# klasmodin/quflow

Measured on AMD Instinct MI355X. Metric: isospectral timesteps/sec at N=1024 (1 GPU) + ensemble steps/sec at 1/2/4/8 GPUs, higher is better.
Workload: dtype f64

## Files before the change

quflow_amd/csrc/api_isomp.hip:

```cpp
#include <cmath>
#include <cstdarg>
#include <cstdio>
#include <cstdlib>
#include <cstring>
#include <limits>
#include <chrono>
#include <type_traits>
#include <utility>

#include "qf_api.h"

namespace {

#ifndef QF_RUN_AHEAD
#define QF_RUN_AHEAD 3
#endif

template <class S> constexpr bool is_c64 = std::is_same<S, qf_c64>::value;

template <class S> S *ws(qf_ctx *ctx)
{
    if constexpr (is_c64<S>) return ctx->c64;
    else return ctx;
}
// ... 92 lines not shown

int select_second_product_c64(qf_ctx *ctx)
{
    qf_c64 *f = ctx->c64;
    f->tri = false;
    if (f->tri_allowed && ctx->gemm_tri_allowed && (qf_c64_tile(ctx) == 32 || ctx->N % 64 == 0) && ctx->N >= 64) {
        QF_TRY(check_skew(ctx, f));
        if (f->w_skew_known) {
            QF_TRY(qf_c64_tri_alloc(ctx));
            f->tri = true;
        }
    }
    return QF_OK;
}

bool triangle_product(const qf_ctx *ctx) { return (ctx->gemm_tri || ctx->gemm_tri32) && (!ctx->gemm_i8 || ctx->gemm_i8_first); }
bool triangle_product(const qf_c64 *f) { return f->tri; }

template <class S> int begin_increment(qf_ctx *ctx, S *w, bool carry)
{
    const size_t mbytes = (size_t)ctx->N * ctx->N * sizeof(*w->W);
    if (carry) {
        if (w->dw_cur != 0)
            QF_HIP(hipMemcpyAsync(w->dW[0], w->dW[w->dw_cur], mbytes, hipMemcpyDeviceToDevice, ctx->stream));
        QF_TRY(qf_launch_lincomb(ctx, 1, w->W, 1, w->dW[0], 0, w->Whalf));
    } else {
        QF_HIP(hipMemsetAsync(w->dW[0], 0, mbytes, ctx->stream));
        QF_HIP(hipMemcpyAsync(w->Whalf, w->W, mbytes, hipMemcpyDeviceToDevice, ctx->stream));
    }
    return QF_OK;
}

template <class S> int enqueue_iterations(qf_ctx *ctx, int step, int first, int count, double vareps)
// ... 35 lines not shown
    d.ticket = ctx->ticket + 402;
    return d;
}

template <class S> int enqueue_iterations_fused(qf_ctx *ctx, int step, int first, int count, double vareps, bool last_step)
{
    S *w = ws<S>(ctx);
    const bool defer = !is_c64<S> && ctx->defer;
    const qf_decide dec = defer ? deferred_decision(ctx) : qf_decide();
    for (int i = first; i < first + count; ++i) {
        qf_guard g;
        g.state = ctx->state;
        g.step = step;
        g.iter = i;
        g.alt = w->Whalf2;
        {
            prof_scope p(ctx, QF_KERNEL_POISSON);
            if constexpr (is_c64<S>) QF_TRY(launch_solve(ctx, w->Whalf, w->Phalf, vareps, g));
            else QF_TRY(launch_solve(ctx, w->Whalf, w->Phalf, vareps, g, defer ? &dec : nullptr));
        }
        {
            prof_scope p(ctx, QF_KERNEL_GEMM1);
            QF_TRY(launch_gemm(ctx, w->Phalf, w->Whalf, w->PW, nullptr, g));
        }
        {
            prof_scope p(ctx, QF_KERNEL_GEMM2);
            const auto ep = epilogue_of(w, true);
            g.alt = nullptr;
            if constexpr (is_c64<S>) {
                if (w->tri) QF_TRY(qf_launch_cgemm_tri(ctx, w->PW, w->Phalf, &ep, g));
                else QF_TRY(qf_launch_cgemm(ctx, w->PW, w->Phalf, nullptr, &ep, g));
            } else {
                QF_TRY(qf_launch_zgemm(ctx, w->PW, w->Phalf, nullptr, &ep, g));
            }
        }
    }
    if (defer && last_step && count > 0) QF_TRY(qf_launch_decide(ctx, dec));
    return QF_OK;
}

int enqueue_iterations_fused_i8(qf_ctx *ctx, int step, int first, int count, double vareps)
{
// ... 66 lines not shown
            jobs.j[0].X = ctx->PW;
            jobs.j[0].planes = ctx->oz_planes[3];
            jobs.j[0].scale = ctx->oz_scale[3];
            QF_TRY(qf_launch_oz_slice(ctx, jobs, g, ctx->oz_digits2));
        }
        {
            prof_scope p(ctx, QF_KERNEL_GEMM2);
            const qf_epilogue ep = epilogue_of(ctx, true);
            QF_TRY(qf_launch_oz_gemm(ctx, ctx->oz_planes[3], ctx->oz_scale[3], ctx->oz_planes[0], ctx->oz_scale[0], nullptr,
                                     &ep, g, ctx->oz_digits2, ctx->oz_digits2 ? ctx->oz_digits : 0));
        }
    }
    return QF_OK;
}

template <class S> struct fused_run {
    qf_ctx *ctx = nullptr;
    int steps = 0, minit = 1, maxit = 1;
    double vareps = 0.0;
    int pred = 1, pred0 = 1;
    std::vector<int> enq_iters;
    int known = 0, enq = 0;
    bool first_seen = false;
    bool aborted = false;
    unsigned long long idle_polls = 0;

    int enqueue(int step, int first, int count)
    {
        if constexpr (!is_c64<S>)
            if (ctx->gemm_i8) return enqueue_iterations_fused_i8(ctx, step, first, count, vareps);
        return enqueue_iterations_fused<S>(ctx, step, first, count, vareps, step == steps - 1);
    }
    bool cold_start = true;
    void begin(qf_ctx *c, int steps_, int minit_, int maxit_, double vareps_)
    {
        ctx = c;
        cold_start = ws<S>(c)->increment_is_zero;
        steps = steps_;
        minit = minit_;
        maxit = maxit_;
        vareps = vareps_;
        pred = ctx->pred_iters;
        if (pred < minit) pred = minit;
        if (pred > maxit) pred = maxit;
        pred0 = ctx->pred_first_iters > 0 ? ctx->pred_first_iters : pred + 1;
        if (pred0 < pred) pred0 = pred;
        if (pred0 > maxit) pred0 = maxit;
        enq_iters.assign((size_t)steps + 1, 0);
        known = enq = 0;
        first_seen = false;
        aborted = false;
        idle_polls = 0;
    }
    bool done() const { return known >= steps; }
    int pump()
    {
        if (done()) return QF_OK;
        while (enq < steps && enq - known < QF_RUN_AHEAD) {
            const int n = (enq == 0 && cold_start) ? pred0 : pred;
            QF_TRY(enqueue(enq, 0, n));
            enq_iters[enq] = n;
            ++enq;
        }
        volatile qf_host_record *rec = ctx->host_rec;
        unsigned long long p = __atomic_load_n(&rec->progress, __ATOMIC_ACQUIRE);
        int ps = (int)(p >> 32), pi = (int)(p & 0xffffffffull);
        if (ps >= QF_STEP_ABORTED) {
            aborted = true;
            known = steps;
            return QF_OK;
        }
        if (!(ps > known || (ps == known && pi >= enq_iters[known]))) {
            if (++idle_polls > (1ull << 22)) {
                QF_HIP(hipStreamSynchronize(ctx->stream));
                p = __atomic_load_n(&rec->progress, __ATOMIC_ACQUIRE);
                ps = (int)(p >> 32);
                pi = (int)(p & 0xffffffffull);
                if (ps >= QF_STEP_ABORTED) {
// ... 16 lines not shown
                first_seen = true;
                if (it >= minit && it <= maxit) ctx->pred_first_iters = it;
            } else if (it >= minit && it <= maxit) {
                pred = it;
            }
            known = ps < enq ? ps : enq;
            if (done()) ctx->pred_iters = pred;
            return QF_OK;
        }
        const int have = enq_iters[known];
        if (have >= maxit) {
            qf_set_error("qf_isomp: step %d did not close after maxit=%d iterations (internal error)", known, maxit);
            return QF_ERR_STATE;
        }
        QF_TRY(enqueue(known, have, maxit - have));
        enq_iters[known] = maxit;
        enq = known + 1;
        if (pred < maxit) pred += 1;
        return QF_OK;
    }
};

bool poll_yields()
{
    static const int mode = [] {
        const char *e = getenv("QUFLOW_HIP_POLL");
        return (e && strcmp(e, "yield") == 0) ? 1 : 0;
    }();
    return mode == 1;
}

inline void poll_relax()
{
    if (poll_yields()) {
// ... 56 lines not shown
int reset_after_abort(qf_ctx *ctx)
{
    if (!ctx->needs_reset) return QF_OK;
    QF_HIP(hipMemsetAsync(ctx->ticket, 0, 704 * sizeof(unsigned), ctx->stream));
    if (ctx->sk_flags) QF_HIP(hipMemsetAsync(ctx->sk_flags + (ctx->sk_slots > 0 ? ctx->sk_slots : ctx->num_cus), 0, 16 * sizeof(unsigned), ctx->stream));
    if (ctx->t32_arrive) {
        const size_t nt = (size_t)(ctx->N + 31) / 32;
        QF_HIP(hipMemsetAsync(ctx->t32_arrive, 0, nt * (nt + 1) / 2 * sizeof(unsigned), ctx->stream));
    }
    if (ctx->c64 && ctx->c64->tri_arrive)
        QF_HIP(hipMemsetAsync(ctx->c64->tri_arrive, 0, ctx->c64->tri_arrive_count * sizeof(unsigned), ctx->stream));
    ctx->needs_reset = false;
    return QF_OK;
}

template <class S> int fused_enter(qf_ctx *ctx, double dt, double tol, int minit, int maxit, bool carry)
{
    S *w = ws<S>(ctx);
    const size_t mbytes = (size_t)ctx->N * ctx->N * sizeof(*w->W);
    const bool tol_on_device = tol < 0;
    const double tol_factor = tol_on_device ? mach_eps<S>(true) * dt / qf_hbar(ctx->N) : 0.0;
    QF_TRY(reset_after_abort(ctx));
    if constexpr (is_c64<S>) {
        QF_TRY(select_second_product_c64(ctx));
    } else {
        QF_TRY(select_second_product(ctx));
        ctx->defer = ctx->defer_allowed && !ctx->gemm_i8 && ctx->gemm_tri32 && ctx->N <= 512;
    }
    w->increment_is_zero = !carry;
    w->increment_valid = true;
    volatile qf_host_record *rec = ctx->host_rec;
    rec->progress = 0ull;
    rec->step_index = 0;
    rec->fault = 0;
    rec->nonfinite = 0;
    __atomic_thread_fence(__ATOMIC_SEQ_CST);
    if (is_c64<S> || carry) {
        if (tol_on_device) QF_TRY(qf_launch_norm_inf(ctx, w->W, ctx->scalars));
        QF_TRY(begin_increment(ctx, w, carry));
        QF_TRY(qf_launch_state_init(ctx, tol, minit, maxit, tol_on_device ? ctx->scalars : nullptr, tol_factor));
    } else {
        QF_TRY(qf_launch_call_begin(ctx, tol, minit, maxit, tol_on_device ? 1 : 0, tol_factor));
    }
    if (!w->W2) QF_HIP(hipMalloc((void **)&w->W2, mbytes));
    if (!w->Whalf2) QF_HIP(hipMalloc((void **)&w->Whalf2, mbytes));
    if constexpr (!is_c64<S>)
        if (ctx->gemm_i8) QF_TRY(qf_oz_alloc(ctx));
    return QF_OK;
}

template <class S> int fused_leave(qf_ctx *ctx, int steps, qf_isomp_stats *stats_out)
{
    S *w = ws<S>(ctx);
    volatile qf_host_record *rec = ctx->host_rec;
    const int w_parity = steps > 0 ? rec->w_parity : 0, wh_sel = steps > 0 ? rec->wh_sel : 0;
    w->dw_cur = steps > 0 ? rec->dw_parity : 0;
    if (w_parity) std::swap(w->W, w->W2);
    if (wh_sel) std::swap(w->Whalf, w->Whalf2);
    if (triangle_product(w) && steps > 0) {
        QF_TRY(qf_launch_mirror_lower(ctx, w->W));
        QF_TRY(qf_launch_mirror_lower(ctx, w->dW[w->dw_cur]));
    }
    if constexpr (!is_c64<S>)
        if (ctx->diag_at_exit) {
            QF_TRY(qf_enqueue_diagnostics(ctx));
            ctx->diag_valid = true;
        }
    QF_HIP(hipStreamSynchronize(ctx->stream));
    if (rec->nonfinite) {
        qf_set_error("array must not contain infs or NaNs");
        ctx->needs_reset = true;
        w->increment_valid = false;
        ctx->diag_valid = false;
        rec->nonfinite = 0;
        return QF_ERR_NONFINITE;
    }
    if (steps > 0 && rec->step_index != steps) {
        qf_set_error("qf_isomp: device completed %d of %d steps (internal error)", rec->step_index, steps);
        return QF_ERR_STATE;
    }
// ... 46 lines not shown
    auto now = [] { return std::chrono::steady_clock::now(); };
    auto ms_since = [&](std::chrono::steady_clock::time_point t) {
        return std::chrono::duration<double, std::milli>(now() - t).count();
    };
    const auto t_entry = now();
    double t_tol = 0, t_sel = 0, t_init = 0, t_loop = 0, t_waitmax = 0, t_waitat = 0, t_enqmax = 0, t_enqat = 0;
    int waitstep = -1, enqstep = -1;
    S *w = ws<S>(ctx);
    const int N = ctx->N;
    const size_t mbytes = (size_t)N * N * sizeof(*w->W);
    const double hb = qf_hbar(N);
    const double vareps = dt / (2 * hb);
    const bool carry = carry_increment && w->increment_valid && !reinitialize;

    if (ctx->fused_allowed && !compsum && !reinitialize) {
        int rc = fused_enter<S>(ctx, dt, tol, minit, maxit, carry);
        t_init = ms_since(t_entry);
        if (rc == QF_OK) rc = run_fused<S>(ctx, steps, minit, maxit, vareps);
        const double t_run = ms_since(t_entry);
        if (rc == QF_OK) rc = fused_leave<S>(ctx, steps, stats_out);
        if (rc != QF_OK) fused_abort(ctx);
        if (dbg)
            fprintf(stderr, "[quflow_hip] %s %d steps (fused step end): init %.3f run %.3f end %.3f ms (cumulative); %lld iterations\n",
                    is_c64<S> ? "qf_c64_isomp" : "qf_isomp", steps, t_init, t_run, ms_since(t_entry),
                    (long long)ctx->host_rec->total_iterations);
        return rc;
    }

    if (tol < 0) {
        double nrm = 0.0;
        QF_TRY(qf_launch_norm_inf(ctx, w->W, ctx->scalars));
// ... 154 lines not shown
        for (int q = 0; q < k; ++q) {
            const int rc = isomp_impl<S>(ctxs[q], dt, steps, tol, minit, maxit, 0, 0, stats_out ? stats_out + q : nullptr, false);
            if (rc != QF_OK) {
                mark_failed(q);
                if (first_rc == QF_OK) first_rc = rc;
            }
        }
        return first_rc;
    }
    auto abort_all = [&](int rc) {
        for (int q = 0; q < k; ++q) fused_abort(ctxs[q]);
        return rc;
    };
    std::vector<fused_run<S>> runs((size_t)k);
    for (int r = 0; r < k; ++r) {
        const int rc = fused_enter<S>(ctxs[r], dt, tol, minit, maxit, false);
        if (rc != QF_OK) return abort_all(rc);
        runs[r].begin(ctxs[r], steps, minit, maxit, dt / (2 * qf_hbar(ctxs[r]->N)));
    }
    for (;;) {
        bool all = true;
        for (int r = 0; r < k; ++r) {
            if (runs[r].done()) continue;
            const int rc = runs[r].pump();
            if (rc != QF_OK) return abort_all(rc);
            all = all && runs[r].done();
        }
        if (all) break;
        poll_relax();
    }
    int first_rc = QF_OK;
// ... 35 lines not shown
    } else {
        QF_TRY(qf_launch_cgemm(ctx, f->PW, f->Phalf, nullptr, &ep));
        QF_TRY(qf_launch_sum_rowpart(ctx, f->rowpart, f->rowpart_tiles, ctx->rowsum));
    }
    QF_HIP(hipMemcpyAsync(dW_new_host, f->dW[1], bytes, hipMemcpyDeviceToHost, ctx->stream));
    QF_HIP(hipMemcpyAsync(Whalf_new_host, f->Whalf, bytes, hipMemcpyDeviceToHost, ctx->stream));
    QF_HIP(hipMemcpyAsync(rowsum_host, ctx->rowsum, (size_t)N * sizeof(double), hipMemcpyDeviceToHost, ctx->stream));
    QF_HIP(hipStreamSynchronize(ctx->stream));
    return QF_OK;
}

}

int qf_rowpart_slots(const qf_ctx *ctx) { return ctx->gemm_tri ? ctx->N / 64 : ctx->gemm_tri32 ? (ctx->N + 31) / 32 : ctx->rowpart_tiles; }

int qf_enqueue_diagnostics(qf_ctx *ctx)
{
    QF_TRY(qf_launch_solve(ctx, ctx->poisson, ctx->W, ctx->stage, 1.0, 1));
    QF_TRY(qf_launch_inner2(ctx, ctx->W, ctx->stage, ctx->scalars + 2));
    QF_HIP(hipMemcpyAsync(ctx->host_scalars, ctx->scalars + 2, 2 * sizeof(double), hipMemcpyDeviceToHost, ctx->stream));
    return QF_OK;
}

int qf_isomp_multi(qf_ctx **ctxs, int k, double dt, int steps, double tol, int minit, int maxit, qf_isomp_stats *stats_out)
{
    return isomp_multi<qf_ctx>(ctxs, k, dt, steps, tol, minit, maxit, stats_out);
}

int qf_c64_isomp_multi(qf_ctx **ctxs, int k, double dt, int steps, double tol, int minit, int maxit, qf_isomp_stats *stats_out)
{
    return isomp_multi<qf_c64>(ctxs, k, dt, steps, tol, minit, maxit, stats_out);
}

int qf_isomp(qf_ctx *ctx, double dt, int steps, double tol, int minit, int maxit, int compsum,
// ... 135 lines not shown
```

quflow_amd/csrc/elementwise.hip:

```cpp
#include "qf_internal.h"

#pragma clang fp contract(off)

namespace {

constexpr int TU = 32;

__device__ __forceinline__ cplx make_c(double re, double im) { return make_double2(re, im); }
__device__ __forceinline__ float2 make_c(float re, float im) { return make_float2(re, im); }
__device__ __forceinline__ double modulus_d(cplx z) { return hypot(z.x, z.y); }
__device__ __forceinline__ double modulus_d(float2 z) { return (double)hypotf(z.x, z.y); }
__device__ __forceinline__ double re_dot_d(cplx a, cplx b) { return a.x * b.x + a.y * b.y; }
__device__ __forceinline__ double re_dot_d(float2 a, float2 b) { return (double)(a.x * b.x + a.y * b.y); }

__device__ void qf_step_advance(qf_dev_state *state, qf_host_record *rec, const qf_guard &guard)
{
    const bool mine = state->step_index == guard.step;
    const bool complete = mine && (state->step_done != 0 || state->iters_this_step >= state->maxit);
    int incomplete = 0;
    if (complete) {
        if (!state->step_done) state->number_of_maxit += 1;
        rec->last_step_iters = state->iters_this_step;
        state->step_index += 1;
        state->iters_this_step = 0;
// ... 174 lines not shown
    const int bi = blockIdx.y, bj = blockIdx.x;
    if (bj > bi) return;
    const int i0 = bi * TU, j0 = bj * TU;
    for (int r = ty; r < TU; r += 8) {
        const int gj = j0 + r, gi = i0 + tx;
        C tv = make_c(R(0), R(0));
        if (gj < N && gi < N) tv = X[(size_t)gj * N + gi];
        Ts[r][tx] = tv;
    }
    __syncthreads();
    for (int r = ty; r < TU; r += 8) {
        const int gi = i0 + r, gj = j0 + tx;
        if (gi < N && gj < N && gj < gi) {
            const C t = Ts[tx][r];
            X[(size_t)gi * N + gj] = make_c(-t.x, t.y);
        }
    }
}

__global__ __launch_bounds__(256) void k_magnetic_fix(int N, const cplx *__restrict__ BTP, const cplx *__restrict__ BT,
                                                       cplx *__restrict__ dW, const cplx *__restrict__ dW_old,
                                                       const cplx *__restrict__ W, cplx *__restrict__ Whalf,
                                                       double *__restrict__ rowpart)
{
    __shared__ cplx Tp[TU][TU + 1], Tb[TU][TU + 1];
    __shared__ double rs[8][TU];
    const int tx = threadIdx.x & 31, ty = threadIdx.x >> 5;
    const int i0 = blockIdx.y * TU, j0 = blockIdx.x * TU;
    for (int r = ty; r < TU; r += 8) {
        const int gj = j0 + r, gi = i0 + tx;
// ... 272 lines not shown
    __hip_atomic_store(&rec->seq, 0ull, __ATOMIC_RELEASE, __HIP_MEMORY_SCOPE_SYSTEM);
}

__device__ __forceinline__ bool last_block_of_launch(unsigned *t, int bid, int nb)
{
    const int g = bid >> 5, ng = (nb + 31) >> 5;
    const int gsize = (g == ng - 1) ? nb - (g << 5) : 32;
    asm volatile("s_waitcnt vmcnt(0)" ::: "memory");
    if (__hip_atomic_fetch_add(t + 1 + g, 1u, __ATOMIC_RELAXED, __HIP_MEMORY_SCOPE_AGENT) != (unsigned)(gsize - 1)) return false;
    __hip_atomic_store(t + 1 + g, 0u, __ATOMIC_RELAXED, __HIP_MEMORY_SCOPE_AGENT);
    if (__hip_atomic_fetch_add(t, 1u, __ATOMIC_RELAXED, __HIP_MEMORY_SCOPE_AGENT) != (unsigned)(ng - 1)) return false;
    __hip_atomic_store(t, 0u, __ATOMIC_RELAXED, __HIP_MEMORY_SCOPE_AGENT);
    return true;
}

__global__ __launch_bounds__(256) void k_call_begin(int N, const cplx *__restrict__ W, cplx *__restrict__ dW0,
                                                     cplx *__restrict__ Whalf, double *__restrict__ rowsum, unsigned *ticket,
                                                     qf_dev_state *state, qf_host_record *rec, double tol, int minit,
                                                     int maxit, int auto_tol, double tol_factor)
{
    __shared__ double part[4];
    __shared__ int last;
    for (int i = blockIdx.x; i < N; i += gridDim.x) {
        double s = 0.0;
        for (int j0 = threadIdx.x; j0 < N; j0 += 4 * 256) {
            cplx z[4];
#pragma unroll
            for (int u = 0; u < 4; ++u) {
                const int j = j0 + u * 256;
                z[u] = make_double2(0.0, 0.0);
                if (j < N) z[u] = W[(size_t)i * N + j];
            }
#pragma unroll
            for (int u = 0; u < 4; ++u) {
                const int j = j0 + u * 256;
                if (j < N) {
                    const size_t e = (size_t)i * N + j;
                    s += hypot(z[u].x, z[u].y);
                    dW0[e] = make_double2(0.0, 0.0);
                    Whalf[e] = z[u];
                }
            }
        }
        s = wave_sum(s);
        __syncthreads();
        if ((threadIdx.x & 63) == 0) part[threadIdx.x >> 6] = s;
        __syncthreads();
        if (threadIdx.x == 0)
            __hip_atomic_store(rowsum + i, (part[0] + part[1]) + (part[2] + part[3]), __ATOMIC_RELAXED, __HIP_MEMORY_SCOPE_AGENT);
    }
    if (threadIdx.x == 0) last = last_block_of_launch(ticket, blockIdx.x, gridDim.x) ? 1 : 0;
    __syncthreads();
    if (!last) return;
    double m = 0.0;
    bool nan = false;
// ... 144 lines not shown
    }
}

}

int qf_launch_mhd_sums(qf_ctx *ctx, const cplx *W, const cplx *P, const cplx *Theta, double *part, double *out_dev)
{
    const size_t n = (size_t)ctx->N * ctx->N;
    int blocks = (int)((n + 255) / 256);
    if (blocks > 1024) blocks = 1024;
    hipLaunchKernelGGL(k_mhd_sums, dim3(blocks), dim3(256), 0, ctx->stream, ctx->N, W, P, Theta, part, ctx->ticket + 640, out_dev);
    QF_HIP(hipGetLastError());
    return QF_OK;
}

int qf_launch_call_begin(qf_ctx *ctx, double tol, int minit, int maxit, int auto_tol, double tol_factor)
{
    hipLaunchKernelGGL(k_call_begin, dim3(ctx->N < 1024 ? ctx->N : 1024), dim3(256), 0, ctx->stream, ctx->N, ctx->W, ctx->dW[0], ctx->Whalf, ctx->rowsum,
                       ctx->ticket + 600, ctx->state, ctx->host_rec, tol, minit, maxit, auto_tol, tol_factor);
    QF_HIP(hipGetLastError());
    return QF_OK;
}

template <class C> int qf_launch_inner2(qf_ctx *ctx, const C *A, const C *B, double *out_dev)
{
    const size_t n = (size_t)ctx->N * ctx->N;
    int blocks = (int)((n + 255) / 256);
    if (blocks > 1024) blocks = 1024;
    hipLaunchKernelGGL(k_inner2<C>, dim3(blocks), dim3(256), 0, ctx->stream, n, A, B, ctx->scalars + 64, ctx->ticket + 640, out_dev);
    QF_HIP(hipGetLastError());
    return QF_OK;
}

template <class C>
// ... 173 lines not shown
```

quflow_amd/csrc/qf_api.h:

```cpp
#pragma once

#include "qf_internal.h"

#include <sched.h>

namespace {
int drain_events(qf_ctx *ctx);

struct prof_scope {
    qf_ctx *ctx;
    qf_event_pair ev;
    bool active;
    prof_scope(qf_ctx *c, int id) : ctx(c), active(((c->profile_mask >> id) & 1) != 0)
    {
        ctx->plan_role = id;
        if (!active) return;
        if ((ctx->prof_seen[id]++ % ctx->profile_stride) != 0) {
            active = false;
            return;
        }
        if (ctx->events_free.empty()) {
            if (hipEventCreate(&ev.start) != hipSuccess || hipEventCreate(&ev.stop) != hipSuccess) {
                active = false;
                return;
// ... 49 lines not shown

int read_scalar(qf_ctx *ctx, const double *dev, double *out)
{
    QF_HIP(hipMemcpyAsync(ctx->host_scalars, dev, sizeof(double), hipMemcpyDeviceToHost, ctx->stream));
    QF_HIP(hipStreamSynchronize(ctx->stream));
    *out = ctx->host_scalars[0];
    return QF_OK;
}

}

extern "C" {
int qf_need_c64(qf_ctx *ctx);
int qf_oz_alloc(qf_ctx *ctx);
int qf_rowpart_slots(const qf_ctx *ctx);
int qf_enqueue_diagnostics(qf_ctx *ctx);
}
```

quflow_amd/csrc/qf_internal.h:

```cpp
#pragma once

#include <hip/hip_runtime.h>

#include <atomic>
#include <cstdarg>
#include <cstdio>
#include <map>
#include <mutex>
#include <string>
#include <vector>

#include "../../include/quflow_hip.h"

typedef double2 cplx;

hipError_t qf_guard_malloc(void **p, size_t bytes);
hipError_t qf_guard_free(void *p);
#define hipMalloc(p, n) qf_guard_malloc((void **)(p), (n))
#define hipFree(p) qf_guard_free((void *)(p))

void qf_set_error(const char *fmt, ...);
struct qf_ctx;
inline void qf_plan_note(qf_ctx *ctx, unsigned long long key, const char *fmt, ...) __attribute__((format(printf, 3, 4)));

// ... 331 lines not shown
    long long slab_budget = 0;
    double *slab = nullptr;
    size_t slab_cap = 0;
    qf_sht sht;
    qf_eigh_ws eigh;
    qf_geom_ws geom;

    double *rowpart = nullptr;
    int rowpart_tiles = 0;
    double *rowsum = nullptr;
    double *scalars = nullptr;
    double *host_scalars = nullptr;
    qf_dev_state *state = nullptr;
    qf_host_record *host_rec = nullptr;
    bool diag_at_exit = false, diag_valid = false;
    unsigned *ticket = nullptr;
    int pred_iters = 3;
    bool gemm_tri_allowed = true;
    bool gemm_tri = false;
    int gemm_tri_min_n = 960;
    bool gemm_tri32 = false;
    int tri32_split = 2, tri32_split_diag = 1;
    cplx *t32_partial = nullptr;
    unsigned *t32_arrive = nullptr;
    bool defer_allowed = true;
    bool defer = false;
    int num_cus = 0;
    cplx *sk_partial = nullptr;
    unsigned *sk_flags = nullptr;
    int sk_slots = 0;
// ... 73 lines not shown

struct qf_epilogue {
    const cplx *PW = nullptr;
    const cplx *W = nullptr;
    cplx *dW[2] = {nullptr, nullptr};
    cplx *Whalf = nullptr;
    double *rowpart = nullptr;
    int fused = 0;
    cplx *Wpair[2] = {nullptr, nullptr};
    cplx *Whalf_step = nullptr;
    unsigned *ticket = nullptr;
    int n_tiles = 0;
    qf_dev_state *state_rw = nullptr;
    qf_host_record *rec = nullptr;
    int debug_drop = 0;
};
struct qf_streamk {
    cplx *partial = nullptr;
    unsigned *flags = nullptr;
    unsigned epoch = 0;
    int *fault = nullptr;
    unsigned *ticket = nullptr;
    int n_tiles = 0;
    qf_dev_state *state_rw = nullptr;
    qf_host_record *rec = nullptr;
    unsigned spin_limit = 1u << 22;
    int debug_drop = 0;
    int slots = 0;
};
struct qf_tri32 {
// ... 71 lines not shown
int qf_launch_oz_gemm(qf_ctx *ctx, const signed char *pa, const double *sa, const signed char *pm, const double *sm,
                      cplx *C, const qf_epilogue *ep = nullptr, qf_guard guard = qf_guard(), int digits = 0, int digits_m = 0,
                      const double *diag = nullptr);

template <class T> struct qf_same_type { typedef T type; };
template <class T> using qf_same = typename qf_same_type<T>::type;
template <class C>
int qf_launch_update(qf_ctx *ctx, const C *PW, C *W, const C *dW_a, const C *dW_b, C *Whalf, qf_same<C> *kahan_c,
                     int reinitialize, qf_guard guard = qf_guard());
int qf_launch_debug_modulus(qf_ctx *ctx, int n, const double *er, const double *ei, double *out_mod, double *out_sqrt);
int qf_launch_norm_from_rowpart(qf_ctx *ctx, const double *rowpart, int tiles, double *out_dev);
int qf_launch_fold_nonfinite(qf_ctx *ctx, const double *in_dev, double *acc_dev);
int qf_launch_norm_decide(qf_ctx *ctx, const double *rowpart, int tiles, qf_guard guard);
int qf_launch_state_init(qf_ctx *ctx, double tol, int minit, int maxit, const double *norm_dev = nullptr, double tol_factor = 0.0);
template <class C> int qf_launch_norm_inf(qf_ctx *ctx, const C *A, double *out_dev);
int qf_launch_call_begin(qf_ctx *ctx, double tol, int minit, int maxit, int auto_tol, double tol_factor);
template <class C> int qf_launch_inner2(qf_ctx *ctx, const C *A, const C *B, double *out_dev);
int qf_launch_inner(qf_ctx *ctx, const cplx *A, const cplx *B, double *out_dev);
int qf_launch_mhd_sums(qf_ctx *ctx, const cplx *W, const cplx *P, const cplx *Theta, double *part, double *out_dev);
int qf_launch_erk_stage(qf_ctx *ctx, const cplx *A, const cplx *B, double inv_hb, const cplx *W, cplx *acc,
                        double c_acc, cplx *Wp, double c_wp, cplx *Wout, double c_fin);
int qf_launch_magnetic_fix(qf_ctx *ctx, const cplx *BTP, const cplx *BT, cplx *dW, const cplx *dW_old, const cplx *W,
                           cplx *Whalf, double *rowpart);
int qf_launch_magnetic_update(qf_ctx *ctx, const cplx *BT, cplx *W, const cplx *dW, cplx *Whalf);
template <class C>
int qf_launch_lincomb(qf_ctx *ctx, double a, const C *X, double b, const qf_same<C> *Y, double c, C *out);
int qf_launch_neg_conj_transpose(qf_ctx *ctx, const cplx *X, cplx *out);
template <class C> int qf_launch_mirror_lower(qf_ctx *ctx, C *X);
int qf_launch_sum_rowpart(qf_ctx *ctx, const double *rowpart, int tiles, double *rowsum_dev);
template <class C> int qf_launch_skew_defect(qf_ctx *ctx, const C *A, double *out_dev);
```

quflow_amd/csrc/zgemm.hip:

```cpp
#include "qf_internal.h"
#include "qf_step_end.h"

#include <cstring>

typedef double v4d __attribute__((ext_vector_type(4)));

#ifdef QF_STAMP
__device__ unsigned long long *qf_stamp_buf = nullptr;
#define QF_STAMP_SLOTS 80
#ifdef QF_STAMP_LIGHT
#define QF_STAMP_AT(slot_)
#define QF_STAMP_PH(kt_, ph_)
__device__ unsigned long long *qf_phase_buf = nullptr;
#else
#define QF_STAMP_AT(slot_)                                                              \
    if (qf_stamp_buf && lane == 0 && (slot_) < QF_STAMP_SLOTS)                          \
        qf_stamp_buf[((size_t)blockIdx.x * (T / 64) + wave) * QF_STAMP_SLOTS + (slot_)] = __builtin_amdgcn_s_memtime();
__device__ unsigned long long *qf_phase_buf = nullptr;
#define QF_STAMP_PH(kt_, ph_)                                                           \
    if (qf_phase_buf && tid == 0 && (kt_) >= 20 && (kt_) < 28)                          \
        qf_phase_buf[((size_t)blockIdx.x * 8 + ((kt_) - 20)) * 5 + (ph_)] = __builtin_amdgcn_s_memtime();
#endif
__device__ unsigned long long *qf_tri_buf = nullptr;
#define QF_TRI_STAMP(seg_, k_)                                                          \
// ... 180 lines not shown
            e_c[mi][ni][reg].y = e_c[mi][ni][reg].y + e_t[mi][ni][reg].y;              \
        }                                                                              \
    }
#define QF_EPI_FETCH(dst_, src_, TRANSPOSED_)                                          \
    {                                                                                  \
        _Pragma("unroll") for (int mi = 0; mi < MT; ++mi)                              \
            _Pragma("unroll") for (int ni = 0; ni < NT; ++ni)                          \
                _Pragma("unroll") for (int reg = 0; reg < 4; ++reg)                    \
        {                                                                              \
            const int gi = i0 + wm * WTM + mi * 16 + q4 + 4 * reg;                     \
            const int gj = j0 + wn * WTN + ni * 16 + r16;                              \
            dst_[mi][ni][reg] = zero;                                                  \
            if (EXACT || (gi < N && gj < N))                                           \
                dst_[mi][ni][reg] = (TRANSPOSED_) ? (src_)[(size_t)gj * N + gi] : (src_)[(size_t)gi * N + gj]; \
        }                                                                              \
    }

    v4d accR[MT][NT], accI[MT][NT], accS[MT][NT];
#pragma unroll
    for (int a = 0; a < MT; ++a)
#pragma unroll
        for (int b = 0; b < NT; ++b) {
            accR[a][b] = (v4d){0.0, 0.0, 0.0, 0.0};
            accI[a][b] = (v4d){0.0, 0.0, 0.0, 0.0};
            accS[a][b] = (v4d){0.0, 0.0, 0.0, 0.0};
        }

    cplx ra[2][A_PER], rb[2][B_PER];
    cplx fa[2][MT], fb[2][NT];
    double fas[2][MT], fbs[2][NT];
// ... 288 lines not shown
        QF_KTILE_STEADY(5, 1, 0)
        kt = 6;
    }
    for (; kt + ((QF_TAIL_STEADY_HERE) ? 1 : 4) < KT; kt += 2) {
        QF_KTILE_STEADY(kt, 0, 0)
        QF_KTILE_STEADY(kt + 1, 1, 0)
    }
    QF_KLOOP_TAIL(kt)
    if (EPI) {
        if (!spread) {
            QF_EPI_FETCH(e_c, ep.PW, false)
            QF_EPI_FETCH(e_t, ep.PW, true)
            QF_EPI_COMM
        }
        QF_EPI_FETCH(e_w, ep_W, false)
        QF_EPI_FETCH(e_old, ep_dW_old, false)
    }

    if constexpr (!EPI) {
#if QF_WT_PW
        const __amdgpu_buffer_rsrc_t rsrcC = __builtin_amdgcn_make_buffer_rsrc(C, 0, 0x7fffffff, 0x00020000);
#endif
#pragma unroll
        for (int mi = 0; mi < MT; ++mi)
#pragma unroll
            for (int ni = 0; ni < NT; ++ni)
#pragma unroll
                for (int reg = 0; reg < 4; ++reg) {
                    int gi = i0 + wm * WTM + mi * 16 + q4 + 4 * reg;
                    int gj = j0 + wn * WTN + ni * 16 + r16;
                    const double cre = accR[mi][ni][reg] - accI[mi][ni][reg];
// ... 257 lines not shown
                                                               p_voff + (unsigned)(((mi * NT + ni) * 4 + reg) * T * sizeof(cplx)),
                                                               (unsigned)((size_t)park_slot * (BM * BN) * sizeof(cplx)), QF_SK_AUX_ST);
                    }
            asm volatile("s_waitcnt vmcnt(0)" ::: "memory");
            if (have_next) QF_TRI_START_LOADS(n_k0, n_KT, n_tm, n_tn)
            __syncthreads();
            if (tid == 0 && !(sk.debug_drop & 1)) __hip_atomic_store(sk.flags + park_slot, sk.epoch, __ATOMIC_RELAXED, __HIP_MEMORY_SCOPE_AGENT);
            QF_TRI_STAMP(seg, 2)
        } else {
            if (!spread) {
                QF_EPI_FETCH(e_c, ep.PW, false)
                QF_EPI_FETCH(e_t, ep.PW, true)
                QF_EPI_COMM
            }
            QF_EPI_FETCH(e_w, ep_W, false)
            QF_EPI_FETCH(e_old, ep_dW_old, false)
            double tre[MT][NT][4], tim[MT][NT][4];
#pragma unroll
            for (int mi = 0; mi < MT; ++mi)
#pragma unroll
                for (int ni = 0; ni < NT; ++ni)
#pragma unroll
                    for (int reg = 0; reg < 4; ++reg) {
                        tre[mi][ni][reg] = accR[mi][ni][reg] - accI[mi][ni][reg];
                        tim[mi][ni][reg] = (accS[mi][ni][reg] - accR[mi][ni][reg]) - accI[mi][ni][reg];
                    }
            if (KT < KTN) {
                const int tile_org = t * S, tile_end = tile_org + S;
                const int c_first = c + 1;
                int c_last = c;
                while (c_last + 1 < G && (int)((long long)(c_last + 1) * U / G) < tile_end) ++c_last;
// ... 289 lines not shown
        QF_KTILE_STEADY(4, 0, 3)
        QF_KTILE_STEADY(5, 1, 0)
        kt = 6;
    }
    for (; kt + ((QF_TAIL_STEADY_HERE) ? 1 : 4) < KT; kt += 2) {
        QF_KTILE_STEADY(kt, 0, 0)
        QF_KTILE_STEADY(kt + 1, 1, 0)
    }
    QF_KLOOP_TAIL(kt)
    if (!spread) {
        QF_EPI_FETCH(e_c, ep.PW, false)
        QF_EPI_FETCH(e_t, ep.PW, true)
        QF_EPI_COMM
    }
    QF_EPI_FETCH(e_w, ep_W, false)
    QF_EPI_FETCH(e_old, ep_dW_old, false)

    double tre[4], tim[4];
#pragma unroll
    for (int reg = 0; reg < 4; ++reg) {
        tre[reg] = accR[0][0][reg] - accI[0][0][reg];
        tim[reg] = (accS[0][0][reg] - accR[0][0][reg]) - accI[0][0][reg];
    }
    unsigned *flagw = reinterpret_cast<unsigned *>(smem_raw + 2 * TT_BYTES + (WN * BM + WM * BN) * sizeof(double));
    if (nh > 1) {
        const __amdgpu_buffer_rsrc_t rsrcP = __builtin_amdgcn_make_buffer_rsrc(sx.partial, 0, 0x7fffffff, 0x00020000);
        const unsigned p_voff = (unsigned)(tid * sizeof(cplx));
        const unsigned slot_bytes = (unsigned)(BM * BN * sizeof(cplx));
#pragma unroll
        for (int reg = 0; reg < 4; ++reg) {
            const cplx v = make_double2(tre[reg], tim[reg]);
// ... 130 lines not shown
            }
        }
    }
    if (ep.fused && !sx.deferred) {
        unsigned *last_flag = reinterpret_cast<unsigned *>(rs);
        if (tid == 0) *last_flag = (ticket_old == (unsigned)(sx.n_tiles - 1)) ? 1u : 0u;
        asm volatile("s_waitcnt lgkmcnt(0)\n\ts_barrier" ::: "memory");
        if (*last_flag != 0u)
            qf_fused_step_end(N, nt, ep.rowpart, sx.ticket, sx.state_rw, sx.rec, guard.iter, tid, reinterpret_cast<double *>(smem_raw));
    }
}

#undef QF_KTILE_STEADY
#undef QF_KTILE_TAIL
#undef QF_KTILE_LAST
#undef QF_KTILE
#undef QF_KTILE_SPREAD
#undef QF_KTILE_PHASE1
#undef QF_STORE_A
#undef QF_STORE_B
#undef QF_EPI_FETCH
#undef QF_EPI_COMM
#undef QF_LOAD_TILE
#undef QF_STORE_TILE
#undef QF_READ_FRAGS
#undef QF_MFMA

struct gemm_cfg {
    int BM, BN;
};
// ... 171 lines not shown
```

Measured before the change: 2695.

## Skip call-entry fills and enqueue exit mirror early to trim per-call overhead

On a cold fused call, the begin kernel no longer zeroes dW0 or copies W into Whalf. The first iteration instead reads W directly, and the GEMM epilogue treats the old increment as zero rather than fetching it. The lower-triangle mirror and diagnostics move into a single device-gated exit kernel, queued right after the last step is enqueued, so they overlap the host polling loop instead of running after it. This removes two full-matrix memory passes per call and some serialized host-side launches, at the cost of more state flags and branches that must stay consistent across the carry, c64 and i8 paths.

```diff
diff --git a/quflow_amd/csrc/api_isomp.hip b/quflow_amd/csrc/api_isomp.hip
--- a/quflow_amd/csrc/api_isomp.hip
+++ b/quflow_amd/csrc/api_isomp.hip
@@ -130,9 +130,6 @@
     return QF_OK;
 }
 
-bool triangle_product(const qf_ctx *ctx) { return (ctx->gemm_tri || ctx->gemm_tri32) && (!ctx->gemm_i8 || ctx->gemm_i8_first); }
-bool triangle_product(const qf_c64 *f) { return f->tri; }
-
 template <class S> int begin_increment(qf_ctx *ctx, S *w, bool carry)
 {
     const size_t mbytes = (size_t)ctx->N * ctx->N * sizeof(*w->W);
@@ -198,18 +195,22 @@
         g.step = step;
         g.iter = i;
         g.alt = w->Whalf2;
+        bool lean = false;
+        if constexpr (!is_c64<S>) lean = ctx->lean_entry && step == 0 && i == 0;
+        auto *Whalf = lean ? w->W : w->Whalf;
         {
             prof_scope p(ctx, QF_KERNEL_POISSON);
-            if constexpr (is_c64<S>) QF_TRY(launch_solve(ctx, w->Whalf, w->Phalf, vareps, g));
-            else QF_TRY(launch_solve(ctx, w->Whalf, w->Phalf, vareps, g, defer ? &dec : nullptr));
+            if constexpr (is_c64<S>) QF_TRY(launch_solve(ctx, Whalf, w->Phalf, vareps, g));
+            else QF_TRY(launch_solve(ctx, Whalf, w->Phalf, vareps, g, defer ? &dec : nullptr));
         }
         {
             prof_scope p(ctx, QF_KERNEL_GEMM1);
-            QF_TRY(launch_gemm(ctx, w->Phalf, w->Whalf, w->PW, nullptr, g));
+            QF_TRY(launch_gemm(ctx, w->Phalf, Whalf, w->PW, nullptr, g));
         }
         {
             prof_scope p(ctx, QF_KERNEL_GEMM2);
-            const auto ep = epilogue_of(w, true);
+            auto ep = epilogue_of(w, true);
+            if constexpr (!is_c64<S>) ep.old_zero = lean ? 1 : 0;
             g.alt = nullptr;
             if constexpr (is_c64<S>) {
                 if (w->tri) QF_TRY(qf_launch_cgemm_tri(ctx, w->PW, w->Phalf, &ep, g));
@@ -306,6 +307,16 @@
     return QF_OK;
 }
 
+bool triangle_product(const qf_ctx *ctx) { return (ctx->gemm_tri || ctx->gemm_tri32) && (!ctx->gemm_i8 || ctx->gemm_i8_first); }
+bool triangle_product(const qf_c64 *f) { return f->tri; }
+
+int enqueue_call_exit(qf_ctx *ctx, int steps)
+{
+    if (triangle_product(ctx)) QF_TRY(qf_launch_call_exit(ctx, ctx->W, ctx->W2, ctx->dW[0], ctx->dW[1], steps));
+    if (ctx->diag_at_exit) QF_TRY(qf_enqueue_diagnostics(ctx, (steps & 1) ? ctx->W2 : ctx->W));
+    return QF_OK;
+}
+
 template <class S> struct fused_run {
     qf_ctx *ctx = nullptr;
     int steps = 0, minit = 1, maxit = 1;
@@ -324,6 +335,13 @@
         return enqueue_iterations_fused<S>(ctx, step, first, count, vareps, step == steps - 1);
     }
     bool cold_start = true;
+    int queue_exit()
+    {
+        if (enq < steps || ctx->exit_queued || ctx->exit_in_leave) return QF_OK;
+        QF_TRY(enqueue_call_exit(ctx, steps));
+        ctx->exit_queued = true;
+        return QF_OK;
+    }
     void begin(qf_ctx *c, int steps_, int minit_, int maxit_, double vareps_)
     {
         ctx = c;
@@ -351,9 +369,11 @@
         while (enq < steps && enq - known < QF_RUN_AHEAD) {
             const int n = (enq == 0 && cold_start) ? pred0 : pred;
             QF_TRY(enqueue(enq, 0, n));
+            ctx->exit_queued = false;
             enq_iters[enq] = n;
             ++enq;
         }
+        QF_TRY(queue_exit());
         volatile qf_host_record *rec = ctx->host_rec;
         unsigned long long p = __atomic_load_n(&rec->progress, __ATOMIC_ACQUIRE);
         int ps = (int)(p >> 32), pi = (int)(p & 0xffffffffull);
@@ -400,10 +420,11 @@
             return QF_ERR_STATE;
         }
         QF_TRY(enqueue(known, have, maxit - have));
+        ctx->exit_queued = false;
         enq_iters[known] = maxit;
         enq = known + 1;
         if (pred < maxit) pred += 1;
-        return QF_OK;
+        return queue_exit();
     }
 };
 
@@ -490,7 +511,7 @@
     return QF_OK;
 }
 
-template <class S> int fused_enter(qf_ctx *ctx, double dt, double tol, int minit, int maxit, bool carry)
+template <class S> int fused_enter(qf_ctx *ctx, double dt, int steps, double tol, int minit, int maxit, bool carry)
 {
     S *w = ws<S>(ctx);
     const size_t mbytes = (size_t)ctx->N * ctx->N * sizeof(*w->W);
@@ -505,6 +526,9 @@
     }
     w->increment_is_zero = !carry;
     w->increment_valid = true;
+    ctx->lean_entry = false;
+    ctx->exit_queued = false;
+    ctx->exit_in_leave = is_c64<S> || carry || ctx->gemm_i8;
     volatile qf_host_record *rec = ctx->host_rec;
     rec->progress = 0ull;
     rec->step_index = 0;
@@ -516,7 +540,8 @@
         QF_TRY(begin_increment(ctx, w, carry));
         QF_TRY(qf_launch_state_init(ctx, tol, minit, maxit, tol_on_device ? ctx->scalars : nullptr, tol_factor));
     } else {
-        QF_TRY(qf_launch_call_begin(ctx, tol, minit, maxit, tol_on_device ? 1 : 0, tol_factor));
+        ctx->lean_entry = steps > 0 && !ctx->gemm_i8;
+        QF_TRY(qf_launch_call_begin(ctx, tol, minit, maxit, tol_on_device ? 1 : 0, tol_factor, ctx->lean_entry ? 0 : 1));
     }
     if (!w->W2) QF_HIP(hipMalloc((void **)&w->W2, mbytes));
     if (!w->Whalf2) QF_HIP(hipMalloc((void **)&w->Whalf2, mbytes));
@@ -531,15 +556,20 @@
     volatile qf_host_record *rec = ctx->host_rec;
     const int w_parity = steps > 0 ? rec->w_parity : 0, wh_sel = steps > 0 ? rec->wh_sel : 0;
     w->dw_cur = steps > 0 ? rec->dw_parity : 0;
+    if constexpr (!is_c64<S>) {
+        if (steps > 0 && !ctx->exit_queued && !ctx->exit_in_leave) QF_TRY(enqueue_call_exit(ctx, steps));
+        ctx->exit_queued = false;
+    }
     if (w_parity) std::swap(w->W, w->W2);
     if (wh_sel) std::swap(w->Whalf, w->Whalf2);
-    if (triangle_product(w) && steps > 0) {
+    const bool here = ctx->exit_in_leave;
+    if (here && triangle_product(w) && steps > 0) {
         QF_TRY(qf_launch_mirror_lower(ctx, w->W));
         QF_TRY(qf_launch_mirror_lower(ctx, w->dW[w->dw_cur]));
     }
     if constexpr (!is_c64<S>)
         if (ctx->diag_at_exit) {
-            QF_TRY(qf_enqueue_diagnostics(ctx));
+            if (here || steps == 0) QF_TRY(qf_enqueue_diagnostics(ctx));
             ctx->diag_valid = true;
         }
     QF_HIP(hipStreamSynchronize(ctx->stream));
@@ -616,7 +646,7 @@
     const bool carry = carry_increment && w->increment_valid && !reinitialize;
 
     if (ctx->fused_allowed && !compsum && !reinitialize) {
-        int rc = fused_enter<S>(ctx, dt, tol, minit, maxit, carry);
+        int rc = fused_enter<S>(ctx, dt, steps, tol, minit, maxit, carry);
         t_init = ms_since(t_entry);
         if (rc == QF_OK) rc = run_fused<S>(ctx, steps, minit, maxit, vareps);
         const double t_run = ms_since(t_entry);
@@ -801,7 +831,7 @@
     };
     std::vector<fused_run<S>> runs((size_t)k);
     for (int r = 0; r < k; ++r) {
-        const int rc = fused_enter<S>(ctxs[r], dt, tol, minit, maxit, false);
+        const int rc = fused_enter<S>(ctxs[r], dt, steps, tol, minit, maxit, false);
         if (rc != QF_OK) return abort_all(rc);
         runs[r].begin(ctxs[r], steps, minit, maxit, dt / (2 * qf_hbar(ctxs[r]->N)));
     }
@@ -867,10 +897,11 @@
 
 int qf_rowpart_slots(const qf_ctx *ctx) { return ctx->gemm_tri ? ctx->N / 64 : ctx->gemm_tri32 ? (ctx->N + 31) / 32 : ctx->rowpart_tiles; }
 
-int qf_enqueue_diagnostics(qf_ctx *ctx)
-{
-    QF_TRY(qf_launch_solve(ctx, ctx->poisson, ctx->W, ctx->stage, 1.0, 1));
-    QF_TRY(qf_launch_inner2(ctx, ctx->W, ctx->stage, ctx->scalars + 2));
+int qf_enqueue_diagnostics(qf_ctx *ctx, const cplx *W)
+{
+    if (!W) W = ctx->W;
+    QF_TRY(qf_launch_solve(ctx, ctx->poisson, W, ctx->stage, 1.0, 1));
+    QF_TRY(qf_launch_inner2(ctx, W, ctx->stage, ctx->scalars + 2));
     QF_HIP(hipMemcpyAsync(ctx->host_scalars, ctx->scalars + 2, 2 * sizeof(double), hipMemcpyDeviceToHost, ctx->stream));
     return QF_OK;
 }
diff --git a/quflow_amd/csrc/elementwise.hip b/quflow_amd/csrc/elementwise.hip
--- a/quflow_amd/csrc/elementwise.hip
+++ b/quflow_amd/csrc/elementwise.hip
@@ -212,6 +212,33 @@
         if (gi < N && gj < N && gj < gi) {
             const C t = Ts[tx][r];
             X[(size_t)gi * N + gj] = make_c(-t.x, t.y);
+        }
+    }
+}
+
+__global__ __launch_bounds__(256) void k_call_exit(int N, cplx *__restrict__ W0, cplx *__restrict__ W1, cplx *__restrict__ dW0,
+                                                    cplx *__restrict__ dW1, const qf_dev_state *__restrict__ state, int steps)
+{
+    __shared__ cplx Ts[TU][TU + 1];
+    const int bi = blockIdx.y, bj = blockIdx.x;
+    if (bj > bi) return;
+    const int done = state->step_index;
+    if (done != steps && done < QF_STEP_ABORTED) return;
+    cplx *__restrict__ X = blockIdx.z == 0 ? (state->w_parity ? W1 : W0) : (state->dw_parity ? dW1 : dW0);
+    const int tx = threadIdx.x & 31, ty = threadIdx.x >> 5;
+    const int i0 = bi * TU, j0 = bj * TU;
+    for (int r = ty; r < TU; r += 8) {
+        const int gj = j0 + r, gi = i0 + tx;
+        cplx tv = make_double2(0.0, 0.0);
+        if (gj < N && gi < N) tv = X[(size_t)gj * N + gi];
+        Ts[r][tx] = tv;
+    }
+    __syncthreads();
+    for (int r = ty; r < TU; r += 8) {
+        const int gi = i0 + r, gj = j0 + tx;
+        if (gi < N && gj < N && gj < gi) {
+            const cplx t = Ts[tx][r];
+            X[(size_t)gi * N + gj] = make_double2(-t.x, t.y);
         }
     }
 }
@@ -514,6 +541,7 @@
     return true;
 }
 
+template <bool FILL>
 __global__ __launch_bounds__(256) void k_call_begin(int N, const cplx *__restrict__ W, cplx *__restrict__ dW0,
                                                      cplx *__restrict__ Whalf, double *__restrict__ rowsum, unsigned *ticket,
                                                      qf_dev_state *state, qf_host_record *rec, double tol, int minit,
@@ -537,8 +565,10 @@
                 if (j < N) {
                     const size_t e = (size_t)i * N + j;
                     s += hypot(z[u].x, z[u].y);
-                    dW0[e] = make_double2(0.0, 0.0);
-                    Whalf[e] = z[u];
+                    if (FILL) {
+                        dW0[e] = make_double2(0.0, 0.0);
+                        Whalf[e] = z[u];
+                    }
                 }
             }
         }
@@ -713,10 +743,23 @@
     return QF_OK;
 }
 
-int qf_launch_call_begin(qf_ctx *ctx, double tol, int minit, int maxit, int auto_tol, double tol_factor)
-{
-    hipLaunchKernelGGL(k_call_begin, dim3(ctx->N < 1024 ? ctx->N : 1024), dim3(256), 0, ctx->stream, ctx->N, ctx->W, ctx->dW[0], ctx->Whalf, ctx->rowsum,
-                       ctx->ticket + 600, ctx->state, ctx->host_rec, tol, minit, maxit, auto_tol, tol_factor);
+int qf_launch_call_begin(qf_ctx *ctx, double tol, int minit, int maxit, int auto_tol, double tol_factor, int fill)
+{
+    const dim3 grid(ctx->N < 1024 ? ctx->N : 1024);
+    if (fill)
+        hipLaunchKernelGGL(k_call_begin<true>, grid, dim3(256), 0, ctx->stream, ctx->N, ctx->W, ctx->dW[0], ctx->Whalf, ctx->rowsum,
+                           ctx->ticket + 600, ctx->state, ctx->host_rec, tol, minit, maxit, auto_tol, tol_factor);
+    else
+        hipLaunchKernelGGL(k_call_begin<false>, grid, dim3(256), 0, ctx->stream, ctx->N, ctx->W, ctx->dW[0], ctx->Whalf, ctx->rowsum,
+                           ctx->ticket + 600, ctx->state, ctx->host_rec, tol, minit, maxit, auto_tol, tol_factor);
+    QF_HIP(hipGetLastError());
+    return QF_OK;
+}
+
+int qf_launch_call_exit(qf_ctx *ctx, cplx *W0, cplx *W1, cplx *dW0, cplx *dW1, int steps)
+{
+    const int tiles = (ctx->N + TU - 1) / TU;
+    hipLaunchKernelGGL(k_call_exit, dim3(tiles, tiles, 2), dim3(256), 0, ctx->stream, ctx->N, W0, W1, dW0, dW1, ctx->state, steps);
     QF_HIP(hipGetLastError());
     return QF_OK;
 }
diff --git a/quflow_amd/csrc/qf_api.h b/quflow_amd/csrc/qf_api.h
--- a/quflow_amd/csrc/qf_api.h
+++ b/quflow_amd/csrc/qf_api.h
@@ -87,5 +87,5 @@
 int qf_need_c64(qf_ctx *ctx);
 int qf_oz_alloc(qf_ctx *ctx);
 int qf_rowpart_slots(const qf_ctx *ctx);
-int qf_enqueue_diagnostics(qf_ctx *ctx);
+int qf_enqueue_diagnostics(qf_ctx *ctx, const cplx *W = nullptr);
 }
diff --git a/quflow_amd/csrc/qf_internal.h b/quflow_amd/csrc/qf_internal.h
--- a/quflow_amd/csrc/qf_internal.h
+++ b/quflow_amd/csrc/qf_internal.h
@@ -369,6 +369,7 @@
     qf_dev_state *state = nullptr;
     qf_host_record *host_rec = nullptr;
     bool diag_at_exit = false, diag_valid = false;
+    bool lean_entry = false, exit_queued = false, exit_in_leave = false;
     unsigned *ticket = nullptr;
     int pred_iters = 3;
     bool gemm_tri_allowed = true;
@@ -472,6 +473,7 @@
     qf_dev_state *state_rw = nullptr;
     qf_host_record *rec = nullptr;
     int debug_drop = 0;
+    int old_zero = 0;
 };
 struct qf_streamk {
     cplx *partial = nullptr;
@@ -573,7 +575,7 @@
 int qf_launch_norm_decide(qf_ctx *ctx, const double *rowpart, int tiles, qf_guard guard);
 int qf_launch_state_init(qf_ctx *ctx, double tol, int minit, int maxit, const double *norm_dev = nullptr, double tol_factor = 0.0);
 template <class C> int qf_launch_norm_inf(qf_ctx *ctx, const C *A, double *out_dev);
-int qf_launch_call_begin(qf_ctx *ctx, double tol, int minit, int maxit, int auto_tol, double tol_factor);
+int qf_launch_call_begin(qf_ctx *ctx, double tol, int minit, int maxit, int auto_tol, double tol_factor, int fill);
 template <class C> int qf_launch_inner2(qf_ctx *ctx, const C *A, const C *B, double *out_dev);
 int qf_launch_inner(qf_ctx *ctx, const cplx *A, const cplx *B, double *out_dev);
 int qf_launch_mhd_sums(qf_ctx *ctx, const cplx *W, const cplx *P, const cplx *Theta, double *part, double *out_dev);
@@ -586,5 +588,6 @@
 int qf_launch_lincomb(qf_ctx *ctx, double a, const C *X, double b, const qf_same<C> *Y, double c, C *out);
 int qf_launch_neg_conj_transpose(qf_ctx *ctx, const cplx *X, cplx *out);
 template <class C> int qf_launch_mirror_lower(qf_ctx *ctx, C *X);
+int qf_launch_call_exit(qf_ctx *ctx, cplx *W0, cplx *W1, cplx *dW0, cplx *dW1, int steps);
 int qf_launch_sum_rowpart(qf_ctx *ctx, const double *rowpart, int tiles, double *rowsum_dev);
 template <class C> int qf_launch_skew_defect(qf_ctx *ctx, const C *A, double *out_dev);
diff --git a/quflow_amd/csrc/zgemm.hip b/quflow_amd/csrc/zgemm.hip
--- a/quflow_amd/csrc/zgemm.hip
+++ b/quflow_amd/csrc/zgemm.hip
@@ -218,6 +218,15 @@
             if (EXACT || (gi < N && gj < N))                                           \
                 dst_[mi][ni][reg] = (TRANSPOSED_) ? (src_)[(size_t)gj * N + gi] : (src_)[(size_t)gi * N + gj]; \
         }                                                                              \
+    }
+
+#define QF_EPI_FETCH_OLD                                                               \
+    {                                                                                  \
+        if (ep.old_zero) {                                                             \
+            _Pragma("unroll") for (int mi = 0; mi < MT; ++mi)                          \
+                _Pragma("unroll") for (int ni = 0; ni < NT; ++ni)                      \
+                    _Pragma("unroll") for (int reg = 0; reg < 4; ++reg) e_old[mi][ni][reg] = zero; \
+        } else QF_EPI_FETCH(e_old, ep_dW_old, false)                                   \
     }
 
     v4d accR[MT][NT], accI[MT][NT], accS[MT][NT];
@@ -536,7 +545,7 @@
             QF_EPI_COMM
         }
         QF_EPI_FETCH(e_w, ep_W, false)
-        QF_EPI_FETCH(e_old, ep_dW_old, false)
+        QF_EPI_FETCH_OLD
     }
 
     if constexpr (!EPI) {
@@ -824,7 +833,7 @@
                 QF_EPI_COMM
             }
             QF_EPI_FETCH(e_w, ep_W, false)
-            QF_EPI_FETCH(e_old, ep_dW_old, false)
+            QF_EPI_FETCH_OLD
             double tre[MT][NT][4], tim[MT][NT][4];
 #pragma unroll
             for (int mi = 0; mi < MT; ++mi)
@@ -1144,7 +1153,7 @@
         QF_EPI_COMM
     }
     QF_EPI_FETCH(e_w, ep_W, false)
-    QF_EPI_FETCH(e_old, ep_dW_old, false)
+    QF_EPI_FETCH_OLD
 
     double tre[4], tim[4];
 #pragma unroll
@@ -1305,6 +1314,7 @@
 #undef QF_KTILE_STEADY
 #undef QF_KTILE_TAIL
 #undef QF_KTILE_LAST
+#undef QF_EPI_FETCH_OLD
 #undef QF_KTILE
 #undef QF_KTILE_SPREAD
 #undef QF_KTILE_PHASE1
```

After: 2685. No clear change (-0.4%).
